# Hello1024/shared-tensor

Measured on AMD Instinct MI355X. Metric: async-DP tokens/sec GPT-2-small, higher is better.
Workload: dtype bf16; 1 GPU; model=gpt2-small, global_batch=64, seq_len=1024, parallelism=async-dp1, codec=1bit, n_params=124439808, paramsync=n/a at n_gpus=1 (no links)

## Files before the change

### build.py

```python
#!/usr/bin/env python3
import argparse
import hashlib
import os
import subprocess
import sysconfig

ROOT = os.path.dirname(os.path.abspath(__file__))
CSRC = os.path.join(ROOT, "sharedtensor_amd", "csrc")
OUT = os.path.join(ROOT, "sharedtensor_amd", "_core.so")
BUILD = os.path.join(ROOT, "build")

SOURCES = [
    "codec_cpu.cpp",
    "engine.cpp",
    "rccl_transport.cpp",
    "hip_kernels.hip",
    "grad_clip_kernels.hip",
    "optim_group_kernels.hip",
    "ln_kernels.hip",
    "add_ln_kernels.hip",
    "add_rms_kernels.hip",
    "ce_kernels.hip",
    "ce_opts_kernels.hip",
    "gelu_kernels.hip",
    "bias_grad_kernels.hip",
    "swiglu_kernels.hip",
    "rope_kernels.hip",
    "attn_kernels.hip",
    "bindings.cpp",
]

HEADERS = ["ce_common.h", "common.h", "codec_cpu.h", "device_util.h", "engine.h", "gelu_math.h", "hip_api.h",
           "optim_step.h", "rccl_transport.h"]


def pybind11_include():
    import pybind11
    return pybind11.get_include()


def build(force=False, debug=False, verbose=True):
    os.makedirs(BUILD, exist_ok=True)
    py_inc = sysconfig.get_paths()["include"]
    rocm = os.environ.get("ROCM_PATH", "/opt/rocm")
    hipcc = os.path.join(rocm, "bin", "hipcc")
    cxxflags = [
        "--offload-arch=gfx950",
        "-std=c++20",
        "-O3" if not debug else "-O0",
        "-g" if debug else "",
        "-fPIC",
        "-DSHAMD_WITH_HIP",
        f"-I{CSRC}",
        f"-I{py_inc}",
        f"-I{pybind11_include()}",
        f"-I{rocm}/include",
        "-Wno-unused-result",
        "-fvisibility=hidden",
        "-DNDEBUG" if not debug else "",
        "-parallel-jobs=4",
    ]
    cxxflags = [f for f in cxxflags if f]

    h = hashlib.sha256()
    for f in SOURCES + HEADERS:
        with open(os.path.join(CSRC, f), "rb") as fh:
            h.update(fh.read())
    h.update(" ".join(cxxflags).encode())
    stamp = os.path.join(BUILD, "core.stamp")
    digest = h.hexdigest()
    if not force and os.path.exists(OUT) and os.path.exists(stamp):
        with open(stamp) as fh:
            if fh.read().strip() == digest:
                if verbose:
                    print(f"[build.py] {OUT} up to date")
                return OUT

    objs = []
    procs = []
    for src in SOURCES:
        obj = os.path.join(BUILD, src.replace("/", "_") + ".o")
        objs.append(obj)
        cmd = [hipcc, "-c", os.path.join(CSRC, src), "-o", obj] + cxxflags
        if verbose:
            print("[build.py]", " ".join(cmd))
        procs.append(subprocess.Popen(cmd))
    rc = 0
    for p in procs:
        rc |= p.wait()
    if rc:
        raise RuntimeError("hipcc compilation failed")

    link = [hipcc, "-shared", "-fPIC", "-o", OUT] + objs + [
        f"-L{rocm}/lib", "-lamdhip64", "-lrccl", "-pthread",
        f"-Wl,-rpath,{rocm}/lib",
    ]
    if verbose:
        print("[build.py]", " ".join(link))
    subprocess.check_call(link)
    nm = subprocess.run(["nm", "-C", "-u", OUT], capture_output=True, text=True)
    bad = [l for l in nm.stdout.splitlines() if "shamd::" in l]
    if bad:
        raise RuntimeError("unresolved engine symbols:\n" + "\n".join(bad))
    with open(stamp, "w") as fh:
        fh.write(digest)
    if verbose:
        print(f"[build.py] built {OUT}")
    return OUT


if __name__ == "__main__":
    ap = argparse.ArgumentParser()
    ap.add_argument("--force", action="store_true")
    ap.add_argument("--debug", action="store_true")
    args = ap.parse_args()
    build(force=args.force, debug=args.debug)
```

### sharedtensor_amd/csrc/bindings.cpp

```cpp
#include <pybind11/pybind11.h>
#include <pybind11/stl.h>

#include <array>

#include "codec_cpu.h"
#include "engine.h"
#include "rccl_transport.h"

namespace py = pybind11;
using namespace shamd;

namespace {

py::tuple py_cpu_encode(int codec, uintptr_t delta, int64_t n, double scale_in,
                        uintptr_t payload_out) {
  Codec c = static_cast<Codec>(codec);
  float* d = reinterpret_cast<float*>(delta);
  float scale = scale_in < 0 ? cpu_compute_scale(c, d, n)
                             : static_cast<float>(scale_in);
  cpu_quantize(c, d, n, scale, reinterpret_cast<uint8_t*>(payload_out));
  return py::make_tuple(scale, payload_bytes(c, n));
}

void py_cpu_apply(int codec, uintptr_t payload, int64_t n, double scale,
// ... 255 lines not shown
      .def("start", &Engine::start, py::call_guard<py::gil_scoped_release>())
      .def("add_from", &Engine::add_from,
           py::call_guard<py::gil_scoped_release>())
      .def("copy_to", &Engine::copy_to,
           py::call_guard<py::gil_scoped_release>())
      .def("fused_sgd", &Engine::fused_sgd, py::arg("mom"), py::arg("grad"),
           py::arg("lr"), py::arg("momentum"), py::arg("stream"),
           py::arg("clip_state") = 0, py::arg("groups") = 0,
           py::call_guard<py::gil_scoped_release>())
      .def("fused_sgd_bf16", &Engine::fused_sgd_bf16, py::arg("mom"),
           py::arg("grad"), py::arg("shadow"), py::arg("lr"),
           py::arg("momentum"), py::arg("stream"), py::arg("clip_state") = 0, py::arg("groups") = 0,
           py::call_guard<py::gil_scoped_release>())
      .def("fused_adamw", &Engine::fused_adamw, py::arg("mom"),
           py::arg("vel"), py::arg("grad"), py::arg("grad_bf16"),
           py::arg("shadow"), py::arg("lr"), py::arg("beta1"),
           py::arg("beta2"), py::arg("eps"), py::arg("wd"), py::arg("step"),
           py::arg("stream"), py::arg("clip_state") = 0, py::arg("groups") = 0,
           py::call_guard<py::gil_scoped_release>())
      .def("grad_clip_coef", &Engine::grad_clip_coef, py::arg("grad"),
           py::arg("grad_bf16"), py::arg("n"), py::arg("max_norm"),
           py::arg("scratch"), py::arg("state"), py::arg("stream"),
           py::call_guard<py::gil_scoped_release>())
      .def("notify_dirty", &Engine::notify_dirty)
      .def("close", &Engine::close, py::call_guard<py::gil_scoped_release>())
      .def("is_master", &Engine::is_master)
      .def("listen_port", &Engine::listen_port)
      .def("last_error", &Engine::last_error)
      .def("reconnect_count", &Engine::reconnect_count)
      .def("recent_scales_sent", &Engine::recent_scales_sent)
      .def("recent_scales_recv", &Engine::recent_scales_recv)
      .def("link_stats", [](Engine& e) {
        py::list out;
        for (auto& s : e.link_stats()) {
          py::dict d;
          d["rounds_sent"] = s.rounds_sent;
          d["rounds_recv"] = s.rounds_recv;
          d["bytes_sent"] = s.bytes_sent;
          d["bytes_recv"] = s.bytes_recv;
          d["last_scale_sent"] = s.last_scale_sent;
          d["last_scale_recv"] = s.last_scale_recv;
          d["active"] = s.active;
          d["dead"] = s.dead;
          d["peer"] = s.peer;
          d["rccl"] = s.rccl;
          out.append(d);
        }
        return out;
      });

  py::class_<DevCodec>(m, "DevCodec")
      .def(py::init<int, std::vector<int64_t>, int, bool>(), py::arg("codec"),
           py::arg("sizes"), py::arg("device"), py::arg("delta_bf16") = false)
      .def("reduce_scales", &DevCodec::reduce_scales)
      .def("quantize", &DevCodec::quantize, py::arg("delta"),
           py::arg("scales"), py::arg("payload"), py::arg("stream"),
           py::arg("stats") = 0)
      .def("finalize_scales", &DevCodec::finalize_scales)
      .def("apply", &DevCodec::apply);
  m.def("gpu_add_scatter", &py_gpu_add_scatter, py::arg("src"), py::arg("n"),
        py::arg("alpha"), py::arg("dsts"), py::arg("stream"),
        py::arg("delta_bf16") = false);
  m.def("gpu_fused_sgd", &py_gpu_fused_sgd, py::arg("mom"), py::arg("grad"),
        py::arg("lr"), py::arg("mu"), py::arg("n"), py::arg("dsts"),
        py::arg("stream"), py::arg("delta_bf16") = false,
        py::arg("clip_state") = 0, py::arg("groups") = 0);
  m.def("gpu_fused_sgd_bf16", &py_gpu_fused_sgd_bf16, py::arg("mom"),
        py::arg("grad"), py::arg("shadow"), py::arg("lr"), py::arg("mu"),
        py::arg("n"), py::arg("dsts"), py::arg("stream"),
        py::arg("delta_bf16") = false, py::arg("clip_state") = 0, py::arg("groups") = 0);
  m.def("gpu_fused_adamw", &py_gpu_fused_adamw, py::arg("mom"),
        py::arg("vel"), py::arg("grad"), py::arg("grad_bf16"),
        py::arg("shadow"), py::arg("lr"), py::arg("beta1"), py::arg("beta2"),
        py::arg("eps"), py::arg("wd"), py::arg("inv_bc1"), py::arg("inv_bc2"),
        py::arg("n"), py::arg("dsts"), py::arg("stream"),
        py::arg("delta_bf16") = false, py::arg("clip_state") = 0, py::arg("groups") = 0);
  m.def("gpu_grad_clip_coef", &py_gpu_grad_clip_coef, py::arg("grad"),
        py::arg("grad_bf16"), py::arg("n"), py::arg("max_norm"),
        py::arg("scratch"), py::arg("state"), py::arg("stream"));
  m.attr("GRAD_CLIP_MAX_BLOCKS") = GRAD_CLIP_MAX_BLOCKS;
  m.def("build_group_table", &build_group_table, py::arg("n"),
        py::arg("seg_end"), py::arg("seg_group"), py::arg("lr_scale"),
        py::arg("weight_decay"));
  m.attr("GROUP_MAX_SEGMENTS") = GROUP_MAX_SEGMENTS;
  m.attr("GROUP_TILE") = GROUP_TILE;
  m.attr("GROUP_GRID_BLOCKS") = GROUP_GRID_BLOCKS;
  m.def("gpu_snapshot_capture", &py_gpu_snapshot_capture, py::arg("values"),
        py::arg("delta"), py::arg("out"), py::arg("n"), py::arg("stream"),
        py::arg("delta_bf16") = false);
  m.def("gpu_add_delta_scatter", &py_gpu_add_delta_scatter, py::arg("src"),
        py::arg("n"), py::arg("dsts"), py::arg("stream"),
        py::arg("delta_bf16") = false);
  m.def("rccl_loopback_payload", &rccl_loopback_payload,
        "Self ncclSend/ncclRecv of a real payload on one device (1-rank "
        "comm): executes the non-blocking enqueue ordering + stream polling "
        "the 2-GPU xGMI links use and verifies the moved bytes.");
  m.def("rccl_self_test", &rccl_self_test,
        py::call_guard<py::gil_scoped_release>());

  m.def("gelu_fwd", [](uintptr_t x, uintptr_t y, int64_t n, uintptr_t stream) {
    hip_gelu_fwd(reinterpret_cast<const void*>(x), reinterpret_cast<void*>(y),
                 n, reinterpret_cast<hipStream_t>(stream));
  });
  m.def("gelu_bwd", [](uintptr_t dy, uintptr_t x, uintptr_t dx, int64_t n,
                       uintptr_t stream) {
    hip_gelu_bwd(reinterpret_cast<const void*>(dy),
                 reinterpret_cast<const void*>(x),
                 reinterpret_cast<void*>(dx), n,
                 reinterpret_cast<hipStream_t>(stream));
  });

  m.def("bias_grad_partial_floats", &hip_bias_grad_partial_floats);
  m.def("bias_grad_sweep_rows", &hip_bias_grad_sweep_rows);
  m.def("gelu_bwd_colsum", [](uintptr_t dy, uintptr_t x, uintptr_t dx,
                              uintptr_t db, uintptr_t partial, int64_t R,
                              int64_t C, uintptr_t stream) {
    hip_gelu_bwd_colsum(reinterpret_cast<const void*>(dy),
                        reinterpret_cast<const void*>(x),
                        reinterpret_cast<void*>(dx),
                        reinterpret_cast<void*>(db),
                        reinterpret_cast<float*>(partial), R, C,
                        reinterpret_cast<hipStream_t>(stream));
  });
  m.def("pack3_colsum", [](uintptr_t s0, uintptr_t s1, uintptr_t s2,
                           uintptr_t dst, uintptr_t db, uintptr_t partial,
                           int64_t R, int64_t C, uintptr_t stream) {
    hip_pack3_colsum(reinterpret_cast<const void*>(s0),
                     reinterpret_cast<const void*>(s1),
                     reinterpret_cast<const void*>(s2),
                     reinterpret_cast<void*>(dst),
                     reinterpret_cast<void*>(db),
                     reinterpret_cast<float*>(partial), R, C,
                     reinterpret_cast<hipStream_t>(stream));
  });

  m.def("attn_fwd_causal_hd64",
        [](uintptr_t q, uintptr_t k, uintptr_t v, uintptr_t out, uintptr_t lse,
           int64_t B, int64_t H, int64_t T, std::array<int64_t, 3> q_strides,
           std::array<int64_t, 3> k_strides, std::array<int64_t, 3> v_strides,
           int64_t lse_stride, double scale, uintptr_t stream) {
          hip_attn_fwd_causal_hd64(
              reinterpret_cast<const void*>(q),
              reinterpret_cast<const void*>(k),
              reinterpret_cast<const void*>(v), reinterpret_cast<void*>(out),
              reinterpret_cast<float*>(lse), B, H, T, q_strides.data(),
              k_strides.data(), v_strides.data(), lse_stride,
              static_cast<float>(scale),
              reinterpret_cast<hipStream_t>(stream));
        },
        py::arg("q"), py::arg("k"), py::arg("v"), py::arg("out"),
        py::arg("lse"), py::arg("B"), py::arg("H"), py::arg("T"),
        py::arg("q_strides"), py::arg("k_strides"), py::arg("v_strides"),
        py::arg("lse_stride"), py::arg("scale"), py::arg("stream"));

  m.def("ce_fwd", [](uintptr_t logits, uintptr_t targets, uintptr_t loss,
                     uintptr_t row_m, uintptr_t row_lse, int64_t R, int64_t V,
                     uintptr_t stream) {
    hip_ce_fwd(reinterpret_cast<const void*>(logits),
               reinterpret_cast<const int32_t*>(targets),
               reinterpret_cast<float*>(loss), reinterpret_cast<float*>(row_m),
               reinterpret_cast<float*>(row_lse), R, V,
               reinterpret_cast<hipStream_t>(stream));
  });
  m.def("ce_bwd", [](uintptr_t logits, uintptr_t targets, uintptr_t row_lse,
                     uintptr_t dlogits, uintptr_t gscale_dev, double inv_r,
                     int64_t R, int64_t V, uintptr_t stream,
                     bool skip_if_unit) {
    hip_ce_bwd(reinterpret_cast<const void*>(logits),
               reinterpret_cast<const int32_t*>(targets),
               reinterpret_cast<const float*>(row_lse),
               reinterpret_cast<void*>(dlogits),
               reinterpret_cast<const float*>(gscale_dev),
               static_cast<float>(inv_r), R, V, skip_if_unit,
               reinterpret_cast<hipStream_t>(stream));
  }, py::arg("logits"), py::arg("targets"), py::arg("row_lse"),
     py::arg("dlogits"), py::arg("gscale_dev"), py::arg("inv_r"),
     py::arg("R"), py::arg("V"), py::arg("stream"),
     py::arg("skip_if_unit") = false);
  m.def("ce_fwd_grad", [](uintptr_t logits, uintptr_t targets, uintptr_t loss,
                          uintptr_t row_lse, uintptr_t dlogits, double inv_r,
                          int64_t R, int64_t V, uintptr_t stream) {
    hip_ce_fwd_grad(reinterpret_cast<const void*>(logits),
                    reinterpret_cast<const int32_t*>(targets),
                    reinterpret_cast<float*>(loss),
                    reinterpret_cast<float*>(row_lse),
                    reinterpret_cast<void*>(dlogits),
                    static_cast<float>(inv_r), R, V,
                    reinterpret_cast<hipStream_t>(stream));
  });
  m.def("ce_fwd_grad_max_v", &hip_ce_fwd_grad_max_v);

  m.attr("CE_OPT_STATE_BYTES") = static_cast<int>(sizeof(CeOptState));
  m.def("ce_opts_scan", [](uintptr_t targets, int64_t R, int64_t V,
                           int32_t ignore_index, bool has_ignore,
                           uintptr_t state, uintptr_t stream) {
    hip_ce_opts_scan(reinterpret_cast<const int32_t*>(targets), R, V,
                     CeOpts{ignore_index, has_ignore, 0.f, 0.f},
                     reinterpret_cast<CeOptState*>(state),
                     reinterpret_cast<hipStream_t>(stream));
  }, py::arg("targets"), py::arg("R"), py::arg("V"), py::arg("ignore_index"),
     py::arg("has_ignore"), py::arg("state"), py::arg("stream"));
  m.def("ce_opts_fwd_grad", [](uintptr_t logits, uintptr_t targets,
                               uintptr_t loss, uintptr_t row_lse,
                               uintptr_t dlogits, uintptr_t state, int64_t R,
                               int64_t V, int32_t ignore_index,
                               bool has_ignore, double label_smoothing,
                               double z_loss, uintptr_t stream) {
    hip_ce_opts_fwd_grad(reinterpret_cast<const void*>(logits),
                         reinterpret_cast<const int32_t*>(targets),
                         reinterpret_cast<float*>(loss),
                         reinterpret_cast<float*>(row_lse),
                         reinterpret_cast<void*>(dlogits),
                         reinterpret_cast<const CeOptState*>(state),
                         CeOpts{ignore_index, has_ignore,
                                static_cast<float>(label_smoothing),
                                static_cast<float>(z_loss)},
                         R, V, reinterpret_cast<hipStream_t>(stream));
  }, py::arg("logits"), py::arg("targets"), py::arg("loss"),
     py::arg("row_lse"), py::arg("dlogits"), py::arg("state"), py::arg("R"),
     py::arg("V"), py::arg("ignore_index"), py::arg("has_ignore"),
     py::arg("label_smoothing"), py::arg("z_loss"), py::arg("stream"));
  m.def("ce_opts_fwd", [](uintptr_t logits, uintptr_t targets, uintptr_t loss,
                          uintptr_t row_lse, int64_t R, int64_t V,
                          int32_t ignore_index, bool has_ignore,
                          double label_smoothing, double z_loss,
                          uintptr_t stream) {
    hip_ce_opts_fwd(reinterpret_cast<const void*>(logits),
                    reinterpret_cast<const int32_t*>(targets),
                    reinterpret_cast<float*>(loss),
                    reinterpret_cast<float*>(row_lse),
                    CeOpts{ignore_index, has_ignore,
                           static_cast<float>(label_smoothing),
                           static_cast<float>(z_loss)},
                    R, V, reinterpret_cast<hipStream_t>(stream));
  }, py::arg("logits"), py::arg("targets"), py::arg("loss"),
     py::arg("row_lse"), py::arg("R"), py::arg("V"), py::arg("ignore_index"),
     py::arg("has_ignore"), py::arg("label_smoothing"), py::arg("z_loss"),
     py::arg("stream"));
  m.def("ce_opts_bwd", [](uintptr_t logits, uintptr_t targets,
                          uintptr_t row_lse, uintptr_t dlogits,
                          uintptr_t gscale_dev, uintptr_t state, int64_t R,
                          int64_t V, int32_t ignore_index, bool has_ignore,
                          double label_smoothing, double z_loss,
                          uintptr_t stream, bool skip_if_unit) {
    hip_ce_opts_bwd(reinterpret_cast<const void*>(logits),
                    reinterpret_cast<const int32_t*>(targets),
                    reinterpret_cast<const float*>(row_lse),
                    reinterpret_cast<void*>(dlogits),
                    reinterpret_cast<const float*>(gscale_dev),
                    reinterpret_cast<const CeOptState*>(state),
                    CeOpts{ignore_index, has_ignore,
                           static_cast<float>(label_smoothing),
                           static_cast<float>(z_loss)},
                    R, V, skip_if_unit, reinterpret_cast<hipStream_t>(stream));
  }, py::arg("logits"), py::arg("targets"), py::arg("row_lse"),
     py::arg("dlogits"), py::arg("gscale_dev"), py::arg("state"), py::arg("R"),
     py::arg("V"), py::arg("ignore_index"), py::arg("has_ignore"),
     py::arg("label_smoothing"), py::arg("z_loss"), py::arg("stream"),
     py::arg("skip_if_unit") = false);

  m.def("ln_fwd", [](uintptr_t x, uintptr_t w, uintptr_t b, uintptr_t y,
                     uintptr_t mean, uintptr_t rstd, int64_t R, int C,
                     double eps, uintptr_t stream) {
    hip_ln_fwd(reinterpret_cast<const void*>(x),
               reinterpret_cast<const void*>(w),
               reinterpret_cast<const void*>(b), reinterpret_cast<void*>(y),
               reinterpret_cast<float*>(mean), reinterpret_cast<float*>(rstd),
               R, C, static_cast<float>(eps),
               reinterpret_cast<hipStream_t>(stream));
  });
  m.def("colsum_bf16", [](uintptr_t x, uintptr_t out, int64_t R, int C,
                          uintptr_t stream) {
    hip_colsum_bf16(reinterpret_cast<const void*>(x),
                    reinterpret_cast<float*>(out), R, C,
                    reinterpret_cast<hipStream_t>(stream));
  });
  m.def("swiglu_fwd", [](uintptr_t x1, uintptr_t x3, uintptr_t y, int64_t n,
                         uintptr_t stream) {
    hip_swiglu_fwd(reinterpret_cast<const void*>(x1),
                   reinterpret_cast<const void*>(x3),
                   reinterpret_cast<void*>(y), n,
                   reinterpret_cast<hipStream_t>(stream));
  });
  m.def("swiglu_bwd", [](uintptr_t dy, uintptr_t x1, uintptr_t x3,
                         uintptr_t dx1, uintptr_t dx3, int64_t n,
                         uintptr_t stream) {
    hip_swiglu_bwd(reinterpret_cast<const void*>(dy),
                   reinterpret_cast<const void*>(x1),
                   reinterpret_cast<const void*>(x3),
                   reinterpret_cast<void*>(dx1),
                   reinterpret_cast<void*>(dx3), n,
                   reinterpret_cast<hipStream_t>(stream));
  });
  m.def("rope_qk", [](uintptr_t q, uintptr_t k, uintptr_t q_out,
                      uintptr_t k_out, uintptr_t cos, uintptr_t sin,
                      int64_t B, int64_t Hq, int64_t Hkv, int64_t T,
                      int64_t D, std::array<int64_t, 3> q_strides,
                      std::array<int64_t, 3> k_strides,
                      std::array<int64_t, 3> q_out_strides,
                      std::array<int64_t, 3> k_out_strides, bool inverse,
                      uintptr_t stream) {
    auto st = [](const std::array<int64_t, 3>& a) {
      return RopeStrides{a[0], a[1], a[2]};
    };
    hip_rope_qk(reinterpret_cast<const void*>(q),
                reinterpret_cast<const void*>(k),
// ... 126 lines not shown
```

### sharedtensor_amd/csrc/hip_api.h

```cpp
#pragma once

#include <hip/hip_runtime.h>

#include "common.h"

namespace shamd {

inline int64_t align8(int64_t x) { return (x + 7) & ~int64_t(7); }

struct DevTable {
  int64_t* offs = nullptr;
  int64_t* poffs = nullptr;
  int T = 0;
  int64_t n = 0;
  int64_t pe = 0;
};


void hip_reduce_scales(Codec c, const void* delta, bool delta_bf16,
                       const DevTable& tb, void* reduce_buf, float* scales_out,
                       int sample_stride, hipStream_t s);

void hip_quantize(Codec c, void* delta, bool delta_bf16, const DevTable& tb,
                  const float* scales_dev, uint8_t* payload, hipStream_t s,
// ... 13 lines not shown
void hip_snapshot_capture(const float* values, void* delta, bool delta_bf16,
                          float* out, int64_t n, hipStream_t s);

void hip_add_delta_scatter(const void* src_delta, bool delta_bf16, int64_t n,
                           float* values, void* d1, void* d2, hipStream_t s);

void hip_fused_sgd(float* mom, const float* grad, float lr, float momentum,
                   int64_t n, float* values, void* d1, void* d2, void* d3,
                   bool delta_bf16, hipStream_t s,
                   const ClipState* clip = nullptr);

void hip_fused_sgd_bf16(float* mom, const uint16_t* grad, uint16_t* shadow,
                        float lr, float momentum, int64_t n, float* values,
                        void* d1, void* d2, void* d3, bool delta_bf16,
                        hipStream_t s, const ClipState* clip = nullptr);

void hip_fused_adamw(float* mom, float* vel, const void* grad, bool grad_bf16,
                     uint16_t* shadow, float lr, float beta1, float beta2,
                     float eps, float wd, float inv_bc1, float inv_bc2,
                     int64_t n, float* values, void* d1, void* d2, void* d3,
                     bool delta_bf16, hipStream_t s,
                     const ClipState* clip = nullptr);

void hip_fused_sgd_grouped(float* mom, const float* grad, float lr,
                           float momentum, int64_t n, float* values, void* d1,
                           void* d2, void* d3, bool delta_bf16, hipStream_t s,
                           const ClipState* clip, const void* table);
void hip_fused_sgd_bf16_grouped(float* mom, const uint16_t* grad,
                                uint16_t* shadow, float lr, float momentum,
                                int64_t n, float* values, void* d1, void* d2,
                                void* d3, bool delta_bf16, hipStream_t s,
                                const ClipState* clip, const void* table);
void hip_fused_adamw_grouped(float* mom, float* vel, const void* grad,
                             bool grad_bf16, uint16_t* shadow, float lr,
                             float beta1, float beta2, float eps,
                             float inv_bc1, float inv_bc2, int64_t n,
                             float* values, void* d1, void* d2, void* d3,
                             bool delta_bf16, hipStream_t s,
                             const ClipState* clip, const void* table);

void hip_grad_clip_coef(const void* grad, bool grad_bf16, int64_t n,
                        double max_norm, double* scratch, ClipState* state,
                        hipStream_t s);

void hip_ln_fwd(const void* x, const void* w, const void* b, void* y,
                float* mean, float* rstd, int64_t R, int C, float eps,
                hipStream_t s);
void hip_ln_bwd(const void* dy, const void* x, const void* w,
                const float* mean, const float* rstd, void* dx, float* dgamma,
                float* dbeta, int64_t R, int C, hipStream_t s);

bool hip_add_ln_supported(int C);
int hip_add_ln_max_blocks();
void hip_add_ln_fwd(const void* x, const void* delta, const void* dbias,
                    const void* w, const void* b, void* x_new, void* y,
                    float* mean, float* rstd, int64_t R, int C, float eps,
                    hipStream_t s);
void hip_add_ln_bwd(const void* dy, const void* x_new, const void* w,
                    const float* mean, const float* rstd, const void* d_x_new,
                    void* dx_total, void* dgamma, void* dbeta, void* ddbias,
                    float* partial, int64_t R, int C, hipStream_t s);

void hip_colsum_bf16(const void* x, float* out, int64_t R, int C,
                     hipStream_t s);

void hip_rms_fwd(const void* x, const void* w, void* y, float* rstd,
                 int64_t R, int C, float eps, hipStream_t s);
void hip_rms_bwd(const void* dy, const void* x, const void* w,
                 const float* rstd, void* dx, float* dgamma, int64_t R, int C,
                 hipStream_t s);

bool hip_add_rms_supported(int C);
int hip_add_rms_max_blocks();
void hip_add_rms_fwd(const void* x, const void* delta, const void* w,
                     void* x_new, void* y, float* rstd, int64_t R, int C,
                     float eps, hipStream_t s);
void hip_add_rms_bwd(const void* dy, const void* x_new, const void* w,
                     const float* rstd, const void* d_x_new, void* dx_total,
                     void* dgamma, float* partial, int64_t R, int C,
                     hipStream_t s);

void hip_ce_fwd(const void* logits, const int32_t* targets, float* loss,
                float* row_m, float* row_lse, int64_t R, int64_t V,
                hipStream_t s);
void hip_ce_bwd(const void* logits, const int32_t* targets,
                const float* row_lse, void* dlogits, const float* gscale_dev,
                float inv_r, int64_t R, int64_t V, bool skip_if_unit,
                hipStream_t s);
int64_t hip_ce_fwd_grad_max_v();
void hip_ce_fwd_grad(const void* logits, const int32_t* targets, float* loss,
                     float* row_lse, void* dlogits, float inv_r, int64_t R,
                     int64_t V, hipStream_t s);

struct CeOptState {
  float inv_count;
  uint32_t n_valid;
  uint32_t n_bad;
  uint32_t pad;
};
struct CeOpts {
  int32_t ignore_index;
  bool has_ignore;
  float eps;
  float z;
};
void hip_ce_opts_scan(const int32_t* targets, int64_t R, int64_t V,
                      const CeOpts& o, CeOptState* state, hipStream_t s);
void hip_ce_opts_fwd_grad(const void* logits, const int32_t* targets,
                          float* loss, float* row_lse, void* dlogits,
                          const CeOptState* state, const CeOpts& o, int64_t R,
                          int64_t V, hipStream_t s);
void hip_ce_opts_fwd(const void* logits, const int32_t* targets, float* loss,
                     float* row_lse, const CeOpts& o, int64_t R, int64_t V,
                     hipStream_t s);
void hip_ce_opts_bwd(const void* logits, const int32_t* targets,
                     const float* row_lse, void* dlogits,
                     const float* gscale_dev, const CeOptState* state,
                     const CeOpts& o, int64_t R, int64_t V, bool skip_if_unit,
                     hipStream_t s);

void hip_swiglu_fwd(const void* x1, const void* x3, void* y, int64_t n,
                    hipStream_t s);
void hip_swiglu_bwd(const void* dy, const void* x1, const void* x3, void* dx1,
                    void* dx3, int64_t n, hipStream_t s);

struct RopeStrides {
  int64_t b = 0, h = 0, t = 0;
};
void hip_rope_qk(const void* q, const void* k, void* q_out, void* k_out,
                 const float* cos, const float* sin, int64_t B, int64_t Hq,
                 int64_t Hkv, int64_t T, int64_t D, const RopeStrides& q_in,
                 const RopeStrides& k_in, const RopeStrides& q_os,
                 const RopeStrides& k_os, bool inverse, hipStream_t s);

void hip_gelu_fwd(const void* x, void* y, int64_t n, hipStream_t s);
void hip_gelu_bwd(const void* dy, const void* x, void* dx, int64_t n,
                  hipStream_t s);

int64_t hip_bias_grad_partial_floats(int64_t N);
int64_t hip_bias_grad_sweep_rows(int64_t R, int64_t N, bool pack);
void hip_gelu_bwd_colsum(const void* dy, const void* x, void* dx, void* db,
                         float* partial, int64_t R, int64_t C, hipStream_t s);
void hip_pack3_colsum(const void* s0, const void* s1, const void* s2,
                      void* dst, void* db, float* partial, int64_t R,
                      int64_t C, hipStream_t s);

void hip_attn_fwd_causal_hd64(const void* q, const void* k, const void* v,
                              void* out, float* lse, int64_t B, int64_t H,
                              int64_t T, const int64_t* q_strides,
                              const int64_t* k_strides,
                              const int64_t* v_strides, int64_t lse_stride,
                              float scale, hipStream_t s);

}
```

### sharedtensor_amd/models/gpt2.py

```python
from __future__ import annotations

import math
import os
from dataclasses import dataclass
from typing import Optional

import torch
import torch.nn as nn
import torch.nn.functional as F


@dataclass
class GPT2Config:
    vocab_size: int = 50257
    n_layer: int = 12
    n_head: int = 12
    n_embd: int = 768
    block_size: int = 1024
    dropout: float = 0.0
    ignore_index: Optional[int] = None
    label_smoothing: float = 0.0
    z_loss: float = 0.0

    @classmethod
    def small(cls):
        return cls()

    @classmethod
    def tiny(cls):
        return cls(vocab_size=256, n_layer=2, n_head=2, n_embd=64,
                   block_size=64)


FUSE_PROJ_BIAS = True

FUSE_QKV_BIAS_GRAD = True
FUSE_FC_BIAS_GRAD = False

FUSE_ATTN_FWD = True


def _flag(env: str, default: bool) -> bool:
    v = os.environ.get(env)
    return default if v is None else v == "1"


def _attn_ok(q, k, v) -> bool:
    if not (_flag("SHTENS_FUSED_ATTN", FUSE_ATTN_FWD) and q.is_cuda):
        return False
    from ..ops import fused_attn
    return fused_attn.can_use(q, k, v)


def _bias_grad_ok(flag: bool, which: str, x, lin: nn.Linear) -> bool:
    if not (flag and x.is_cuda and x.dtype == torch.bfloat16
            and lin.bias is not None and torch.is_grad_enabled()):
        return False
    from ..ops import fused_bias_grad as fb
    check = fb.can_use_gelu if which == "gelu" else fb.can_use_qkv
    return check(x, lin.weight, lin.bias)


class FusedLayerNorm(nn.LayerNorm):

    def forward(self, x):
        if (x.is_cuda and x.dtype == torch.bfloat16
                and self.weight.dtype == torch.bfloat16):
            from ..ops import fused_ln
            if fused_ln.can_use(x, self.weight):
                return fused_ln.fused_layer_norm(x, self.weight, self.bias,
                                                 self.eps)
            with torch.autocast("cuda", enabled=False):
                return F.layer_norm(x, self.normalized_shape, self.weight,
                                    self.bias, self.eps)
        return super().forward(x)


def _fused_ln_ok(ln: nn.LayerNorm, x: torch.Tensor) -> bool:
    if (x.is_cuda and x.dtype == torch.bfloat16
            and ln.weight.dtype == torch.bfloat16):
        from ..ops import fused_ln
        return fused_ln.can_use(x, ln.weight)
    return False


def add_ln(ln: nn.LayerNorm, x, delta, delta_bias=None):
    if delta is None:
        return x, ln(x)
    if _fused_ln_ok(ln, x):
        from ..ops import fused_ln
        return fused_ln.fused_add_layer_norm(x, delta, ln.weight, ln.bias,
                                             ln.eps, delta_bias)
    x = x + delta
    if delta_bias is not None:
        x = x + delta_bias
    return x, ln(x)


class CausalSelfAttention(nn.Module):
    def __init__(self, cfg: GPT2Config):
        super().__init__()
        assert cfg.n_embd % cfg.n_head == 0
        self.qkv = nn.Linear(cfg.n_embd, 3 * cfg.n_embd)
        self.proj = nn.Linear(cfg.n_embd, cfg.n_embd)
        self.n_head = cfg.n_head
        self.head_dim = cfg.n_embd // cfg.n_head

    def forward(self, x, proj_bias=True):
        B, T, C = x.shape
        if _bias_grad_ok(_flag("SHTENS_FUSED_QKV_BGRAD", FUSE_QKV_BIAS_GRAD),
                         "qkv", x, self.qkv):
            from ..ops import fused_bias_grad
            qkv = F.linear(x, self.qkv.weight, self.qkv.bias.detach())
            q, k, v = fused_bias_grad.qkv_split_bgrad(qkv, self.qkv.bias)
        else:
            q, k, v = self.qkv(x).split(C, dim=2)
        q = q.view(B, T, self.n_head, self.head_dim).transpose(1, 2)
        k = k.view(B, T, self.n_head, self.head_dim).transpose(1, 2)
        v = v.view(B, T, self.n_head, self.head_dim).transpose(1, 2)
        if _attn_ok(q, k, v):
            from ..ops import fused_attn
            y = fused_attn.fused_causal_attention(q, k, v)
        elif x.is_cuda:
            from torch.nn.attention import SDPBackend, sdpa_kernel
            with sdpa_kernel([SDPBackend.EFFICIENT_ATTENTION,
                              SDPBackend.FLASH_ATTENTION, SDPBackend.MATH],
                             set_priority=True):
                y = F.scaled_dot_product_attention(q, k, v, is_causal=True)
        else:
            y = F.scaled_dot_product_attention(q, k, v, is_causal=True)
        y = y.transpose(1, 2).contiguous().view(B, T, C)
        if not proj_bias:
            return F.linear(y, self.proj.weight)
        return self.proj(y)


class MLP(nn.Module):
    def __init__(self, cfg: GPT2Config):
        super().__init__()
        self.fc = nn.Linear(cfg.n_embd, 4 * cfg.n_embd)
        self.proj = nn.Linear(4 * cfg.n_embd, cfg.n_embd)

    def forward(self, x, proj_bias=True):
        if _bias_grad_ok(_flag("SHTENS_FUSED_GELU_BGRAD", FUSE_FC_BIAS_GRAD),
                         "gelu", x, self.fc):
            from ..ops import fused_bias_grad
            pre = F.linear(x, self.fc.weight, self.fc.bias.detach())
            h = fused_bias_grad.bias_gelu_bgrad(pre, self.fc.bias)
        else:
            h = F.gelu(self.fc(x), approximate="tanh")
        if not proj_bias:
            return F.linear(h, self.proj.weight)
        return self.proj(h)


class Block(nn.Module):
    def __init__(self, cfg: GPT2Config):
        super().__init__()
        self.ln1 = FusedLayerNorm(cfg.n_embd)
        self.attn = CausalSelfAttention(cfg)
        self.ln2 = FusedLayerNorm(cfg.n_embd)
        self.mlp = MLP(cfg)

    def forward(self, x, delta=None, delta_bias=None, fuse_proj_bias=False):
        x, h = add_ln(self.ln1, x, delta, delta_bias)
        fuse = fuse_proj_bias and _fused_ln_ok(self.ln2, x)
        a = self.attn(h, proj_bias=not fuse)
        x, h = add_ln(self.ln2, x, a, self.attn.proj.bias if fuse else None)
        m = self.mlp(h, proj_bias=not fuse)
        return x, m, (self.mlp.proj.bias if fuse else None)


class GPT2(nn.Module):
    def __init__(self, cfg: GPT2Config):
        super().__init__()
        self.cfg = cfg
        self.wte = nn.Embedding(cfg.vocab_size, cfg.n_embd)
        self.wpe = nn.Embedding(cfg.block_size, cfg.n_embd)
        self.blocks = nn.ModuleList(Block(cfg) for _ in range(cfg.n_layer))
        self.ln_f = FusedLayerNorm(cfg.n_embd)
        self.lm_head = nn.Linear(cfg.n_embd, cfg.vocab_size, bias=False)
        self.lm_head.weight = self.wte.weight
        self.apply(self._init)
        for name, p in self.named_parameters():
            if name.endswith("proj.weight"):
                nn.init.normal_(p, std=0.02 / math.sqrt(2 * cfg.n_layer))

    @staticmethod
    def _init(m):
        if isinstance(m, nn.Linear):
            nn.init.normal_(m.weight, std=0.02)
            if m.bias is not None:
                nn.init.zeros_(m.bias)
        elif isinstance(m, nn.Embedding):
            nn.init.normal_(m.weight, std=0.02)

    def forward(self, idx, targets=None):
        B, T = idx.shape
        pos = torch.arange(T, device=idx.device)
        x = self.wte(idx) + self.wpe(pos)
        delta = delta_bias = None
        for blk in self.blocks:
            x, delta, delta_bias = blk(x, delta, delta_bias,
                                       FUSE_PROJ_BIAS)
        _, x = add_ln(self.ln_f, x, delta, delta_bias)
        logits = self.lm_head(x)
        if targets is None:
            return logits, None
        flat = logits.view(-1, logits.size(-1))
        tgt = targets.reshape(-1)
        cfg = self.cfg
        if cfg.ignore_index is not None or cfg.label_smoothing != 0.0 \
                or cfg.z_loss != 0.0:
            from ..ops import fused_ce
            opts = dict(ignore_index=cfg.ignore_index,
                        label_smoothing=cfg.label_smoothing,
                        z_loss=cfg.z_loss)
            if fused_ce.can_use(flat):
                return logits, fused_ce.fused_cross_entropy(flat, tgt, **opts)
            return logits, fused_ce.cross_entropy_reference(flat.float(), tgt,
                                                            **opts)
        if flat.is_cuda and flat.dtype == torch.bfloat16:
            from ..ops import fused_ce
            if fused_ce.can_use(flat):
                return logits, fused_ce.fused_cross_entropy(flat, tgt)
        loss = F.cross_entropy(flat, tgt)
        return logits, loss

    def num_params(self) -> int:
        return sum(p.numel() for p in self.parameters())
```

Measured before the change: 836,600 tokens/s.

## Add custom MFMA weight-gradient kernel for attention linears

```diff
diff --git a/build.py b/build.py
--- a/build.py
+++ b/build.py
@@ -27,6 +27,7 @@
     "swiglu_kernels.hip",
     "rope_kernels.hip",
     "attn_kernels.hip",
+    "wgrad_kernels.hip",
     "bindings.cpp",
 ]
 
diff --git a/sharedtensor_amd/csrc/bindings.cpp b/sharedtensor_amd/csrc/bindings.cpp
--- a/sharedtensor_amd/csrc/bindings.cpp
+++ b/sharedtensor_amd/csrc/bindings.cpp
@@ -431,6 +431,29 @@
         py::arg("lse"), py::arg("B"), py::arg("H"), py::arg("T"),
         py::arg("q_strides"), py::arg("k_strides"), py::arg("v_strides"),
         py::arg("lse_stride"), py::arg("scale"), py::arg("stream"));
+
+  m.def("wgrad_num_variants", &hip_wgrad_num_variants);
+  m.def("wgrad_tile", [](int variant) {
+    int tn = 0, tk = 0;
+    hip_wgrad_tile(variant, &tn, &tk);
+    return std::make_pair(tn, tk);
+  });
+  m.def("wgrad_bf16",
+        [](uintptr_t dy, uintptr_t x, uintptr_t dw, uintptr_t ws,
+           int64_t ws_floats, int64_t M, int64_t N, int64_t K, int64_t ldy,
+           int64_t ldx, int64_t ldw, int64_t split, int variant,
+           uintptr_t stream) {
+          hip_wgrad_bf16(reinterpret_cast<const void*>(dy),
+                         reinterpret_cast<const void*>(x),
+                         reinterpret_cast<void*>(dw),
+                         reinterpret_cast<float*>(ws), ws_floats, M, N, K, ldy,
+                         ldx, ldw, split, variant,
+                         reinterpret_cast<hipStream_t>(stream));
+        },
+        py::arg("dy"), py::arg("x"), py::arg("dw"), py::arg("ws"),
+        py::arg("ws_floats"), py::arg("M"), py::arg("N"), py::arg("K"),
+        py::arg("ldy"), py::arg("ldx"), py::arg("ldw"), py::arg("split"),
+        py::arg("variant"), py::arg("stream"));
 
   m.def("ce_fwd", [](uintptr_t logits, uintptr_t targets, uintptr_t loss,
                      uintptr_t row_m, uintptr_t row_lse, int64_t R, int64_t V,
diff --git a/sharedtensor_amd/csrc/hip_api.h b/sharedtensor_amd/csrc/hip_api.h
--- a/sharedtensor_amd/csrc/hip_api.h
+++ b/sharedtensor_amd/csrc/hip_api.h
@@ -189,4 +189,11 @@
                               const int64_t* v_strides, int64_t lse_stride,
                               float scale, hipStream_t s);
 
+int hip_wgrad_num_variants();
+void hip_wgrad_tile(int variant, int* tile_n, int* tile_k);
+void hip_wgrad_bf16(const void* dy, const void* x, void* dw, float* ws,
+                    int64_t ws_floats, int64_t M, int64_t N, int64_t K,
+                    int64_t ldy, int64_t ldx, int64_t ldw, int64_t split,
+                    int variant, hipStream_t s);
+
 }
diff --git a/sharedtensor_amd/csrc/wgrad_kernels.hip b/sharedtensor_amd/csrc/wgrad_kernels.hip
--- /dev/null
+++ b/sharedtensor_amd/csrc/wgrad_kernels.hip
@@ -0,0 +1,286 @@
+#include <hip/hip_runtime.h>
+
+#include "device_util.h"
+#include "hip_api.h"
+
+namespace shamd {
+namespace {
+
+typedef __bf16 bf16x8 __attribute__((ext_vector_type(8)));
+typedef __bf16 bf16x4 __attribute__((ext_vector_type(4)));
+typedef float f32x16 __attribute__((ext_vector_type(16)));
+typedef short s16x4 __attribute__((ext_vector_type(4)));
+
+constexpr int kStep = 64;
+constexpr int kPanelCols = 128;
+constexpr int kPanelBytes = kStep * kPanelCols * 2;
+constexpr int kXcd = 8;
+
+__device__ __forceinline__ int p_off(int row, int ch) {
+  return row * 256 + ((ch ^ (((row & 3) << 2) | ((row >> 2) & 3))) << 4);
+}
+
+template <int NP, int KP, int NBUF>
+__global__ __launch_bounds__(256 * NP * KP)
+    __attribute__((amdgpu_waves_per_eu(NBUF == 1 ? 3 : 2,
+                                       NBUF == 1 ? 3 : 2))) void k_wgrad(
+    const uint16_t* __restrict__ dy, const uint16_t* __restrict__ x,
+    uint16_t* __restrict__ dw, float* __restrict__ ws, int steps, int N, int K,
+    int64_t ldy, int64_t ldx, int64_t ldw, int split, int tiles_k, int tiles) {
+  constexpr int NT = 256 * NP * KP;
+  constexpr int kStage = (NP + KP) * kPanelBytes;
+  constexpr int kChunks = (NP + KP) * 1024 / NT;
+  static_assert((NP + KP) * 1024 % NT == 0 && 1024 % NT == 0, "staging map");
+  __shared__ __attribute__((aligned(16))) unsigned char lds[NBUF * kStage];
+
+  const int nwg = gridDim.x, orig = blockIdx.x;
+  const int xcd = orig % kXcd, q8 = nwg / kXcd, r8 = nwg % kXcd;
+  const int wg =
+      (xcd < r8 ? xcd * (q8 + 1) : r8 * (q8 + 1) + (xcd - r8) * q8) +
+      orig / kXcd;
+  const int sp = wg / tiles, tile = wg % tiles;
+  const int n0 = (tile / tiles_k) * (kPanelCols * NP);
+  const int k0 = (tile % tiles_k) * (kPanelCols * KP);
+
+  const int sq = steps / split, sr = steps % split;
+  const int s_begin = sp * sq + min(sp, sr);
+  const int s_count = sq + (sp < sr ? 1 : 0);
+
+  const int tid = threadIdx.x;
+  const int wave = __builtin_amdgcn_readfirstlane(tid >> 6), lane = tid & 63;
+  const int wn = wave / (2 * KP), wk = wave % (2 * KP);
+
+  const int srow = (tid & 1023) >> 4, sch = tid & 15;
+  constexpr int kCA = NP * 1024 / NT, kCB = KP * 1024 / NT;
+  static_assert(kCA + kCB == kChunks && kCA <= 4 && kCB <= 4, "staging map");
+  uint4 sa0, sa1, sa2, sa3, sb0, sb1, sb2, sb3;
+  const int64_t tok0 = (int64_t)s_begin * kStep + srow;
+  const uint16_t* const pa = dy + tok0 * ldy + n0 + 8 * sch;
+  const uint16_t* const pb = x + tok0 * ldx + k0 + 8 * sch;
+#define SHAMD_WG_LOAD(reg, i, p, ld, cnt)                                    \
+  if constexpr ((i) < (cnt))                                                 \
+    reg = *reinterpret_cast<const uint4*>(                                   \
+        (p) + (t + ((((i) * NT) & 1023) >> 4)) * (ld) +                      \
+        (((i) * NT) >> 10) * kPanelCols)
+#define SHAMD_WG_STORE(reg, i, p0, cnt)                                      \
+  if constexpr ((i) < (cnt))                                                 \
+    *reinterpret_cast<uint4*>(                                               \
+        base + ((p0) + (((i) * NT) >> 10)) * kPanelBytes +                   \
+        p_off(srow + ((((i) * NT) & 1023) >> 4), sch)) = reg
+  auto issue = [&](int step) {
+    const int64_t t = (int64_t)step * kStep;
+    SHAMD_WG_LOAD(sa0, 0, pa, ldy, kCA);
+    SHAMD_WG_LOAD(sa1, 1, pa, ldy, kCA);
+    SHAMD_WG_LOAD(sa2, 2, pa, ldy, kCA);
+    SHAMD_WG_LOAD(sa3, 3, pa, ldy, kCA);
+    SHAMD_WG_LOAD(sb0, 0, pb, ldx, kCB);
+    SHAMD_WG_LOAD(sb1, 1, pb, ldx, kCB);
+    SHAMD_WG_LOAD(sb2, 2, pb, ldx, kCB);
+    SHAMD_WG_LOAD(sb3, 3, pb, ldx, kCB);
+  };
+  auto commit = [&](int buf) {
+    unsigned char* const base = lds + buf * kStage;
+    SHAMD_WG_STORE(sa0, 0, 0, kCA);
+    SHAMD_WG_STORE(sa1, 1, 0, kCA);
+    SHAMD_WG_STORE(sa2, 2, 0, kCA);
+    SHAMD_WG_STORE(sa3, 3, 0, kCA);
+    SHAMD_WG_STORE(sb0, 0, NP, kCB);
+    SHAMD_WG_STORE(sb1, 1, NP, kCB);
+    SHAMD_WG_STORE(sb2, 2, NP, kCB);
+    SHAMD_WG_STORE(sb3, 3, NP, kCB);
+  };
+#undef SHAMD_WG_LOAD
+#undef SHAMD_WG_STORE
+
+  f32x16 acc[2][2];
+#pragma unroll
+  for (int i = 0; i < 2; ++i)
+#pragma unroll
+    for (int j = 0; j < 2; ++j)
+#pragma unroll
+      for (int e = 0; e < 16; ++e) acc[i][j][e] = 0.f;
+
+  const int grp = lane >> 4, gi = lane & 15;
+  const int tr_q = gi >> 2, tr_p = gi & 3, hi = grp >> 1;
+  const int a_ch = (wn & 1) * 8 + 2 * (grp & 1) + (tr_p >> 1);
+  const int b_ch = (wk & 1) * 8 + 2 * (grp & 1) + (tr_p >> 1);
+  const int a_panel = (wn >> 1) * kPanelBytes;
+  const int b_panel = (NP + (wk >> 1)) * kPanelBytes;
+
+  auto frag = [&](const unsigned char* panel, int ch, int ss) -> bf16x8 {
+    bf16x8 f;
+#pragma unroll
+    for (int jj = 0; jj < 2; ++jj) {
+      const int row = 16 * ss + 8 * jj + 4 * hi + tr_q;
+      auto* a = reinterpret_cast<__attribute__((address_space(3))) s16x4*>(
+          (uintptr_t)(panel + p_off(row, ch) + 8 * (tr_p & 1)));
+      s16x4 tr = __builtin_amdgcn_ds_read_tr16_b64_v4i16(a);
+      bf16x4 tb = __builtin_bit_cast(bf16x4, tr);
+#pragma unroll
+      for (int e = 0; e < 4; ++e) f[4 * jj + e] = tb[e];
+    }
+    return f;
+  };
+  auto compute = [&](int buf) {
+    const unsigned char* A = lds + buf * kStage + a_panel;
+    const unsigned char* B = lds + buf * kStage + b_panel;
+#pragma unroll
+    for (int ss = 0; ss < 4; ++ss) {
+      bf16x8 a[2], b[2];
+#pragma unroll
+      for (int i = 0; i < 2; ++i) {
+        a[i] = frag(A, a_ch + 4 * i, ss);
+        b[i] = frag(B, b_ch + 4 * i, ss);
+      }
+#pragma unroll
+      for (int i = 0; i < 2; ++i)
+#pragma unroll
+        for (int j = 0; j < 2; ++j)
+          acc[i][j] = __builtin_amdgcn_mfma_f32_32x32x16_bf16(
+              a[i], b[j], acc[i][j], 0, 0, 0);
+    }
+  };
+
+  if (s_count > 0) {
+    issue(0);
+    commit(0);
+    __syncthreads();
+    for (int t = 0; t < s_count; ++t) {
+      const bool more = t + 1 < s_count;
+      if (more) issue(t + 1);
+      if constexpr (NBUF == 2) {
+        compute(t & 1);
+        if (more) commit((t & 1) ^ 1);
+        __syncthreads();
+      } else {
+        compute(0);
+        __syncthreads();
+        if (more) commit(0);
+        __syncthreads();
+      }
+    }
+  }
+
+  const int row0 = n0 + wn * 64 + 4 * (lane >> 5);
+  const int col0 = k0 + wk * 64 + (lane & 31);
+  if (split == 1) {
+#pragma unroll
+    for (int i = 0; i < 2; ++i)
+#pragma unroll
+      for (int j = 0; j < 2; ++j)
+#pragma unroll
+        for (int e = 0; e < 16; ++e) {
+          const int row = row0 + 32 * i + (e & 3) + 8 * (e >> 2);
+          dw[(int64_t)row * ldw + col0 + 32 * j] = f32_to_bf16(acc[i][j][e]);
+        }
+  } else {
+    float* out = ws + (int64_t)sp * N * K;
+#pragma unroll
+    for (int i = 0; i < 2; ++i)
+#pragma unroll
+      for (int j = 0; j < 2; ++j)
+#pragma unroll
+        for (int e = 0; e < 16; ++e) {
+          const int row = row0 + 32 * i + (e & 3) + 8 * (e >> 2);
+          out[(int64_t)row * K + col0 + 32 * j] = acc[i][j][e];
+        }
+  }
+}
+
+__global__ __launch_bounds__(256) void k_wgrad_reduce(
+    const float* __restrict__ ws, uint16_t* __restrict__ dw, int64_t groups,
+    int K8, int64_t NK, int64_t ldw, int split) {
+  const int64_t g = (int64_t)blockIdx.x * 256 + threadIdx.x;
+  if (g >= groups) return;
+  const int64_t row = g / K8;
+  const int col = (int)(g % K8) * 8;
+  const float* p = ws + row * (int64_t)(K8 * 8) + col;
+  float v[8];
+  {
+    const float4 a = *reinterpret_cast<const float4*>(p);
+    const float4 b = *reinterpret_cast<const float4*>(p + 4);
+    v[0] = a.x, v[1] = a.y, v[2] = a.z, v[3] = a.w;
+    v[4] = b.x, v[5] = b.y, v[6] = b.z, v[7] = b.w;
+  }
+  for (int s = 1; s < split; ++s) {
+    const float4 a = *reinterpret_cast<const float4*>(p + s * NK);
+    const float4 b = *reinterpret_cast<const float4*>(p + s * NK + 4);
+    v[0] += a.x, v[1] += a.y, v[2] += a.z, v[3] += a.w;
+    v[4] += b.x, v[5] += b.y, v[6] += b.z, v[7] += b.w;
+  }
+  *reinterpret_cast<uint4*>(dw + row * ldw + col) = pack8(v);
+}
+
+struct Variant {
+  int tile_n, tile_k;
+};
+constexpr Variant kVariants[] = {{128, 128}, {128, 128}, {256, 128}};
+constexpr int kNumVariants = sizeof(kVariants) / sizeof(kVariants[0]);
+
+}
+
+int hip_wgrad_num_variants() { return kNumVariants; }
+
+void hip_wgrad_tile(int variant, int* tile_n, int* tile_k) {
+  if (variant < 0 || variant >= kNumVariants)
+    throw std::runtime_error("wgrad_bf16: unknown variant");
+  *tile_n = kVariants[variant].tile_n;
+  *tile_k = kVariants[variant].tile_k;
+}
+
+void hip_wgrad_bf16(const void* dy, const void* x, void* dw, float* ws,
+                    int64_t ws_floats, int64_t M, int64_t N, int64_t K,
+                    int64_t ldy, int64_t ldx, int64_t ldw, int64_t split,
+                    int variant, hipStream_t s) {
+  const char* op = "wgrad_bf16";
+  auto fail = [&](const char* what) {
+    throw std::runtime_error(std::string(op) + ": " + what);
+  };
+  if (variant < 0 || variant >= kNumVariants) fail("unknown variant");
+  const int tn = kVariants[variant].tile_n, tk = kVariants[variant].tile_k;
+  if (M <= 0 || N <= 0 || K <= 0) fail("empty problem");
+  if (M % kStep) fail("M must be a multiple of 64");
+  if (N % tn || K % tk) fail("N and K must be multiples of the tile");
+  if (ldy < N || ldx < K || ldw < K) fail("row stride shorter than the row");
+  if (ldy % 8 || ldx % 8 || ldw % 8)
+    fail("row strides must be multiples of 8 elements");
+  check_align(dy, 16, op, "dy");
+  check_align(x, 16, op, "x");
+  check_align(dw, 16, op, "dw");
+  const int64_t steps = M / kStep;
+  const int64_t tiles = (N / tn) * (K / tk);
+  if (split < 1 || split > 4096) fail("split out of range");
+  if (steps > 0x7fffffff / kStep || N > (1 << 24) || K > (1 << 24) ||
+      tiles * split > 0x7fffffff)
+    fail("problem too large");
+  if (split > 1) {
+    if (ws == nullptr || ws_floats < split * N * K)
+      fail("workspace smaller than split * N * K floats");
+    check_align(ws, 16, op, "ws");
+  }
+  auto* dyp = static_cast<const uint16_t*>(dy);
+  auto* xp = static_cast<const uint16_t*>(x);
+  auto* dwp = static_cast<uint16_t*>(dw);
+  const dim3 grid((unsigned)(tiles * split));
+  const int tiles_k = (int)(K / tk);
+#define SHAMD_WGRAD_LAUNCH(NP, KP, NBUF)                                     \
+  k_wgrad<NP, KP, NBUF><<<grid, dim3(256 * NP * KP), 0, s>>>(                \
+      dyp, xp, dwp, ws, (int)steps, (int)N, (int)K, ldy, ldx, ldw,           \
+      (int)split, tiles_k, (int)tiles)
+  switch (variant) {
+    case 0: SHAMD_WGRAD_LAUNCH(1, 1, 2); break;
+    case 1: SHAMD_WGRAD_LAUNCH(1, 1, 1); break;
+    default: SHAMD_WGRAD_LAUNCH(2, 1, 2); break;
+  }
+#undef SHAMD_WGRAD_LAUNCH
+  HIP_CHECK(hipGetLastError());
+  if (split > 1) {
+    const int64_t groups = N * K / 8;
+    k_wgrad_reduce<<<dim3((unsigned)((groups + 255) / 256)), dim3(256), 0,
+                     s>>>(ws, dwp, groups, (int)(K / 8), N * K, ldw,
+                          (int)split);
+    HIP_CHECK(hipGetLastError());
+  }
+}
+
+}
diff --git a/sharedtensor_amd/models/gpt2.py b/sharedtensor_amd/models/gpt2.py
--- a/sharedtensor_amd/models/gpt2.py
+++ b/sharedtensor_amd/models/gpt2.py
@@ -39,10 +39,20 @@
 
 FUSE_ATTN_FWD = True
 
+FUSE_WGRAD = True
+
 
 def _flag(env: str, default: bool) -> bool:
     v = os.environ.get(env)
     return default if v is None else v == "1"
+
+
+def _linear(x, weight, bias=None):
+    if _flag("SHTENS_FUSED_WGRAD", FUSE_WGRAD) and x.is_cuda:
+        from ..ops import fused_wgrad
+        if fused_wgrad.wired(x, weight):
+            return fused_wgrad.linear_wgrad(x, weight, bias)
+    return F.linear(x, weight, bias)
 
 
 def _attn_ok(q, k, v) -> bool:
@@ -111,10 +121,11 @@
         if _bias_grad_ok(_flag("SHTENS_FUSED_QKV_BGRAD", FUSE_QKV_BIAS_GRAD),
                          "qkv", x, self.qkv):
             from ..ops import fused_bias_grad
-            qkv = F.linear(x, self.qkv.weight, self.qkv.bias.detach())
+            qkv = _linear(x, self.qkv.weight, self.qkv.bias.detach())
             q, k, v = fused_bias_grad.qkv_split_bgrad(qkv, self.qkv.bias)
         else:
-            q, k, v = self.qkv(x).split(C, dim=2)
+            q, k, v = _linear(x, self.qkv.weight,
+                              self.qkv.bias).split(C, dim=2)
         q = q.view(B, T, self.n_head, self.head_dim).transpose(1, 2)
         k = k.view(B, T, self.n_head, self.head_dim).transpose(1, 2)
         v = v.view(B, T, self.n_head, self.head_dim).transpose(1, 2)
@@ -131,8 +142,8 @@
             y = F.scaled_dot_product_attention(q, k, v, is_causal=True)
         y = y.transpose(1, 2).contiguous().view(B, T, C)
         if not proj_bias:
-            return F.linear(y, self.proj.weight)
-        return self.proj(y)
+            return _linear(y, self.proj.weight)
+        return _linear(y, self.proj.weight, self.proj.bias)
 
 
 class MLP(nn.Module):
@@ -145,13 +156,14 @@
         if _bias_grad_ok(_flag("SHTENS_FUSED_GELU_BGRAD", FUSE_FC_BIAS_GRAD),
                          "gelu", x, self.fc):
             from ..ops import fused_bias_grad
-            pre = F.linear(x, self.fc.weight, self.fc.bias.detach())
+            pre = _linear(x, self.fc.weight, self.fc.bias.detach())
             h = fused_bias_grad.bias_gelu_bgrad(pre, self.fc.bias)
         else:
-            h = F.gelu(self.fc(x), approximate="tanh")
+            h = F.gelu(_linear(x, self.fc.weight, self.fc.bias),
+                       approximate="tanh")
         if not proj_bias:
-            return F.linear(h, self.proj.weight)
-        return self.proj(h)
+            return _linear(h, self.proj.weight)
+        return _linear(h, self.proj.weight, self.proj.bias)
 
 
 class Block(nn.Module):
diff --git a/sharedtensor_amd/ops/fused_wgrad.py b/sharedtensor_amd/ops/fused_wgrad.py
--- /dev/null
+++ b/sharedtensor_amd/ops/fused_wgrad.py
@@ -0,0 +1,143 @@
+from __future__ import annotations
+
+from typing import List, Optional, Tuple
+
+import torch
+import torch.nn.functional as F
+
+STEP = 64
+NUM_CU = 256
+
+VARIANTS = {0: (128, 128, 2), 1: (128, 128, 2), 2: (256, 128, 1)}
+DEFAULT_VARIANT = 1
+
+TUNED: dict = {(768, 768): 1, (2304, 768): 1}
+
+
+def split_ranges(steps: int, split: int) -> List[Tuple[int, int]]:
+    if steps < 0 or split < 1:
+        raise ValueError("steps >= 0 and split >= 1")
+    q, r = divmod(steps, split)
+    return [(s * q + min(s, r), q + (1 if s < r else 0)) for s in range(split)]
+
+
+def choose_split(tiles: int, steps: int, per_cu: int,
+                 num_cu: int = NUM_CU) -> int:
+    if tiles < 1 or steps < 1:
+        raise ValueError("tiles >= 1 and steps >= 1")
+    return max(1, min(steps, (num_cu * per_cu) // tiles))
+
+
+def _mat_ok(t: torch.Tensor) -> bool:
+    return (t.dim() == 2 and t.stride(1) == 1 and t.stride(0) % 8 == 0
+            and t.stride(0) >= t.shape[1] and t.data_ptr() % 16 == 0)
+
+
+def can_use(dy: torch.Tensor, x: torch.Tensor,
+            variant: int = DEFAULT_VARIANT) -> bool:
+    if variant not in VARIANTS:
+        return False
+    if not (dy.is_cuda and x.is_cuda and dy.device == x.device):
+        return False
+    if not (dy.dtype == x.dtype == torch.bfloat16):
+        return False
+    if not (_mat_ok(dy) and _mat_ok(x)) or dy.shape[0] != x.shape[0]:
+        return False
+    tn, tk, _ = VARIANTS[variant]
+    M, N, K = dy.shape[0], dy.shape[1], x.shape[1]
+    return M > 0 and M % STEP == 0 and N > 0 and K > 0 \
+        and N % tn == 0 and K % tk == 0
+
+
+_workspace: dict = {}
+
+
+def _workspace_for(device, n: int, stream: int) -> torch.Tensor:
+    key = (device.index, stream)
+    buf = _workspace.get(key)
+    if buf is None or buf.numel() < n:
+        buf = torch.empty(n, dtype=torch.float32, device=device)
+        _workspace[key] = buf
+    return buf
+
+
+def wgrad(dy: torch.Tensor, x: torch.Tensor, out: Optional[torch.Tensor] = None,
+          split: Optional[int] = None, variant: Optional[int] = None,
+          ws: Optional[torch.Tensor] = None) -> torch.Tensor:
+    from .. import _core
+    if variant is None:
+        variant = TUNED.get((dy.shape[1], x.shape[1]), DEFAULT_VARIANT)
+    if not can_use(dy, x, variant):
+        raise ValueError("fused_wgrad: operands the kernel does not take "
+                         "(see can_use)")
+    M, N, K = dy.shape[0], dy.shape[1], x.shape[1]
+    tn, tk, per_cu = VARIANTS[variant]
+    if out is None:
+        out = torch.empty((N, K), dtype=torch.bfloat16, device=dy.device)
+    if (out.shape != (N, K) or out.dtype != torch.bfloat16
+            or out.device != dy.device or not _mat_ok(out)):
+        raise ValueError("fused_wgrad: out must be (N, K) bf16 with unit "
+                         "column stride and an aligned row stride")
+    if split is None:
+        split = choose_split((N // tn) * (K // tk), M // STEP, per_cu)
+    s = torch.cuda.current_stream(dy.device).cuda_stream
+    need = split * N * K if split > 1 else 0
+    if need and ws is None:
+        ws = _workspace_for(dy.device, need, s)
+    if need and (ws.dtype != torch.float32 or not ws.is_contiguous()
+                 or ws.numel() < need or ws.device != dy.device):
+        raise ValueError("fused_wgrad: ws must be contiguous fp32 with at "
+                         "least split * N * K elements")
+    _core.wgrad_bf16(dy.data_ptr(), x.data_ptr(), out.data_ptr(),
+                     ws.data_ptr() if need else 0, ws.numel() if need else 0,
+                     M, N, K, dy.stride(0), x.stride(0), out.stride(0),
+                     split, variant, s)
+    return out
+
+
+def _rows(t: torch.Tensor) -> torch.Tensor:
+    t = t.reshape(-1, t.shape[-1])
+    return t if t.stride(1) == 1 else t.contiguous()
+
+
+class _LinearWgrad(torch.autograd.Function):
+    @staticmethod
+    def forward(ctx, x, weight, bias):
+        ctx.save_for_backward(x, weight)
+        ctx.has_bias = bias is not None
+        return F.linear(x, weight, bias)
+
+    @staticmethod
+    def backward(ctx, dy):
+        x, weight = ctx.saved_tensors
+        dy2, x2 = _rows(dy), _rows(x)
+        dx = dw = db = None
+        with torch.autocast(device_type=dy.device.type, enabled=False):
+            if ctx.needs_input_grad[0]:
+                dx = dy2.to(weight.dtype).mm(weight).to(x.dtype).view(x.shape)
+            if ctx.needs_input_grad[1]:
+                variant = TUNED.get(tuple(weight.shape), DEFAULT_VARIANT)
+                if weight.dtype == torch.bfloat16 and can_use(dy2, x2, variant):
+                    dw = wgrad(dy2, x2, variant=variant)
+                else:
+                    dw = dy2.t().to(weight.dtype).mm(x2.to(weight.dtype))
+            if ctx.has_bias and ctx.needs_input_grad[2]:
+                db = dy2.sum(0)
+        return dx, dw, db
+
+
+def linear_wgrad(x: torch.Tensor, weight: torch.Tensor,
+                 bias: Optional[torch.Tensor] = None) -> torch.Tensor:
+    return _LinearWgrad.apply(x, weight, bias)
+
+
+def wired(x: torch.Tensor, weight: torch.Tensor) -> bool:
+    if not (x.is_cuda and x.dtype == torch.bfloat16
+            and weight.dtype == torch.bfloat16 and weight.dim() == 2
+            and torch.is_grad_enabled() and weight.requires_grad):
+        return False
+    variant = TUNED.get(tuple(weight.shape))
+    if variant is None or x.dim() < 2 or x.shape[-1] != weight.shape[1]:
+        return False
+    M = x.numel() // x.shape[-1]
+    return M > 0 and M % STEP == 0 and x.shape[-1] % 8 == 0
```

New measurement: 855,700 tokens/s (median of 6 runs). +2.3%, better.
